# centreborelli/satnerf

Hardware: AMD Instinct MI355X
Metric: training rays/sec (64 samples/ray) (higher is better)
Workload: dtype bf16; 1 GPU; BASELINE configs[1] sat-nerf 256/tau4, 1024 rays x 64 samples/GPU, mlp_mode=bf16, saved state 8-bit, noise_std=0 sc_lambda=0 n_importance=0, stratified jitter drawn in-kernel (Philox-4x32-10); rays_per_gpu=1024, global_batch=1024, n_samples=64, parallelism=dp1

## Files before the change

include/satrender.h:

```cpp
#ifndef SATRENDER_H
#define SATRENDER_H

#include <stdint.h>

#ifdef __cplusplus
extern "C" {
#endif

#define SR_VERSION 100

#define SR_MODE_BF16 1
#define SR_MODE_BF16X3 3
#define SR_MODE_F16 2

#define SR_FMT16 16
#define SR_FMT8 8

int sr_version(void);
const char* sr_last_error(void);

int64_t sr_fwd_stream_elems(int feat, int tau);
int64_t sr_bwd_stream_elems(int feat, int tau);
int64_t sr_act_elems_per_tile(int feat, int fmt);
int64_t sr_dpre_elems_per_tile(int feat, int fmt);
// ... 49 lines not shown
  int tick;
  const float* noise;
  float noise_std;
  int sky_hidden;
  const float* sky_w1;
  const float* sky_b1;
  const float* sky_w2;
  const float* sky_b2;
  int64_t bank_chunks;
} sr_render_args;

typedef struct sr_render_outputs {
  float* z_vals;
  float* albedo;
  float* sigma;
  float* sun_v;
  float* beta;
  float* sky;
  float* weights;
  float* transparency;
  float* depth;
  float* rgb;
} sr_render_outputs;

int sr_satnerf_render_fwd(const sr_render_args* in, int feat, int tau, int mode, const uint16_t* stream_hi, const uint16_t* stream_lo,
                          const float* l0, const sr_render_outputs* out, void* stream);
int sr_render_points_per_block(int feat, int mode);

typedef struct sr_train_args {
  const float* target;
  const float* sched;
  float beta_min;
  float* loss_parts;
  float* rgb;
  float* d_sigma;
  float* d_albedo;
  float* d_sun_v;
  float* g_beta;
  float* d_sky;
  const int64_t* gather_idx;
  float* cursor;
  int64_t batches;
  float* out_rays;
  float* out_rgbs;
  int64_t* out_ts;
} sr_train_args;
int sr_satnerf_render_train(const sr_render_args* in, int feat, int tau, int mode, const uint16_t* stream_hi, const uint16_t* stream_lo,
                            const float* l0, const sr_render_outputs* out, const sr_train_args* train, uint16_t* acts, int act_fmt, void* stream);

int sr_satnerf_mlp_bwd(int feat, int tau, int64_t n_points, const uint16_t* bwd_stream, const uint16_t* acts,
                       const float* albedo, const float* sigma, const float* sun_v, const float* beta, const float* g_albedo,
                       const float* g_sigma, const float* g_sun_v, const float* g_beta, uint16_t* dpre, float* d_t, int fmt,
                       void* stream);
int sr_wgrad_plan(int32_t* blocks, int n_blocks, int64_t n_points, int n_wg, int fmt, int* n_slices);
int sr_satnerf_wgrad(int feat, int tau, int64_t n_points, const uint16_t* dpre, const uint16_t* acts, const int32_t* blocks,
                     int n_blocks, int n_slices, float* partial, void* stream);
int sr_satnerf_wgrad8(int feat, int tau, int64_t n_points, const uint16_t* dpre, int64_t dpre_elems, const uint16_t* acts,
                      const int32_t* blocks, const int32_t* loads, int n_blocks, int n_slices, int plan_span, float* partial, void* stream);
int sr_wgrad8_load_ints(void);

int sr_sky_bwd(const float* sun, int sun_stride, int64_t n, int hidden, const float* w1, const float* b1, const float* w2,
               const float* sky, const float* d_sky, float* g_w1, float* g_b1, float* g_w2, float* g_b2, void* stream);
int sr_embedding_bwd(const float* d_t, const int64_t* ts, int64_t n_rays, int n_samples, int tau, float* g_emb, void* stream);

int sr_sc_loss(const float* z_vals, const float* sigma, const float* noise, float noise_std, const float* sun_v, int64_t n_rays,
               int n_samples, float lambda_sc, float* loss_parts, float* d_sun_v, void* stream);
int sr_depth_loss(const float* depth, const float* depths, int depths_stride, int use_weights, int64_t n_rays, float lambda_ds,
                  float* loss_parts, float* g_depth, void* stream);
int sr_ray_setup(const float* rays, int ray_stride, const float* u, int64_t n_rays, int n_samples, int hidden, const float* w1,
                 const float* b1, const float* w2, const float* b2, float* z_vals, float* sky, void* stream);
int sr_ray_setup_rng(const float* rays, int ray_stride, uint64_t seed, float* step_counter, int tick, int64_t n_rays, int n_samples,
                     int hidden, const float* w1, const float* b1, const float* w2, const float* b2, float* z_vals, float* sky,
                     void* stream);
int sr_render_loss(const float* z_vals, const float* sigma, const float* noise, float noise_std, const float* albedo,
                   const float* sun_v, const float* beta, const float* sky, const float* target, int64_t n_rays, int n_samples,
                   float beta_min, const float* sched, float* loss_parts, float* rgb, float* d_sigma, float* d_albedo, float* d_sun_v,
                   float* g_beta, float* d_sky, void* stream);

int sr_grad_tail(const float* partial, const int32_t* gidx, const float* gscale, int64_t n_params, const int32_t* blocks, int n_blocks,
                 float* grad, int accumulate, const float* sun, int sun_stride, int64_t n_rays, int hidden,
                 const float* w1, const float* b1, const float* w2, const float* sky, const float* d_sky, float* g_w1, float* g_b1,
                 float* g_w2, float* g_b2, const float* d_t, const int64_t* ts, int n_samples, int tau, float* g_emb, void* stream);
typedef struct sr_pack_scatter {
  const int32_t* map;
  uint16_t* hi;
  uint16_t* lo;
  float* l0;
  int64_t n_f16;
  float scales[4];
} sr_pack_scatter;
int sr_grad_tail_adam(const float* partial, const int32_t* gidx, const float* gscale, int64_t n_params, const int32_t* blocks, int n_blocks,
                      float* grad,
                      int accumulate, const float* sun, int sun_stride, int64_t n_rays, int hidden, const float* w1, const float* b1,
                      const float* w2, const float* sky, const float* d_sky, float* g_w1, float* g_b1, float* g_w2, float* g_b2,
                      const float* d_t, const int64_t* ts, int n_samples, int tau, float* g_emb, float* params, float* exp_avg,
                      float* exp_avg_sq, const int32_t* late_idx, int n_late, float* state, float lr, float beta1, float beta2, float eps,
                      float grad_scale, const sr_pack_scatter* pack, void* stream);
int sr_adam_step_graph(float* params, float* grads, float* exp_avg, float* exp_avg_sq, int64_t n, float lr, float beta1,
                       float beta2, float eps, float grad_scale, float* state, int zero_grad, void* stream);
int sr_adam_step_pack(float* params, float* grads, float* exp_avg, float* exp_avg_sq, int64_t n, float lr, float beta1, float beta2,
                      float eps, float grad_scale, float* state, int zero_grad, int64_t n_packed, const sr_pack_scatter* pack,
                      void* stream);

enum { SR_ACT_NONE = 0, SR_ACT_SIN = 1, SR_ACT_RELU = 2 };
enum { SR_OUT_NONE = 0, SR_OUT_SOFTPLUS = 1, SR_OUT_SIGMOID = 2, SR_OUT_SIGMOID_RGB = 3 };
typedef struct sr_linear_src {
// ... 96 lines not shown
```

satnerf_amd/_lib.py:

```python
from __future__ import annotations

import ctypes as C
import os

_HERE = os.path.dirname(os.path.abspath(__file__))
LIB_PATH = os.environ.get("SATRENDER_LIB") or os.path.join(_HERE, "csrc", "libsatrender.so")

MODE_BF16 = 1
MODE_F16 = 2
MODE_BF16X3 = 3
FMT16, FMT8 = 16, 8

_vp, _i, _i64, _f, _d = C.c_void_p, C.c_int, C.c_int64, C.c_float, C.c_double


class MlpInputs(C.Structure):
    _fields_ = [("org", _vp), ("org_stride", _i), ("dir", _vp), ("dir_stride", _i), ("sun", _vp), ("sun_stride", _i),
                ("z", _vp), ("temb", _vp), ("ts", _vp), ("n_points", _i64), ("n_samples", _i)]


class RenderArgs(C.Structure):
    _fields_ = [("rays", _vp), ("ray_stride", _i), ("ts", _vp), ("temb", _vp), ("n_rays", _i64), ("n_samples", _i), ("z_in", _vp), ("u", _vp),
                ("seed", C.c_uint64), ("step_counter", _vp), ("tick", _i), ("noise", _vp), ("noise_std", _f), ("sky_hidden", _i),
                ("sky_w1", _vp), ("sky_b1", _vp), ("sky_w2", _vp), ("sky_b2", _vp), ("bank_chunks", _i64)]


class RenderOutputs(C.Structure):
    _fields_ = [(k, _vp) for k in ("z_vals", "albedo", "sigma", "sun_v", "beta", "sky", "weights", "transparency", "depth", "rgb")]


class TrainArgs(C.Structure):
    _fields_ = [("target", _vp), ("sched", _vp), ("beta_min", _f), ("loss_parts", _vp), ("rgb", _vp), ("d_sigma", _vp), ("d_albedo", _vp),
                ("d_sun_v", _vp), ("g_beta", _vp), ("d_sky", _vp), ("gather_idx", _vp), ("cursor", _vp), ("batches", _i64), ("out_rays", _vp),
                ("out_rgbs", _vp), ("out_ts", _vp)]


class PackScatter(C.Structure):
    _fields_ = [("map", _vp), ("hi", _vp), ("lo", _vp), ("l0", _vp), ("n_f16", _i64), ("scales", _f * 4)]


class LinearSrc(C.Structure):
    _fields_ = [("x", _vp), ("ld", _i), ("k", _i), ("act", _i), ("w0", _f), ("row_div", _i)]


ACT_NONE, ACT_SIN, ACT_RELU = 0, 1, 2
OUT_NONE, OUT_SOFTPLUS, OUT_SIGMOID, OUT_SIGMOID_RGB = 0, 1, 2, 3

SIGNATURES = {
    "sr_version": (_i, []),
    "sr_last_error": (C.c_char_p, []),
    "sr_fwd_stream_elems": (_i64, [_i, _i]),
    "sr_bwd_stream_elems": (_i64, [_i, _i]),
    "sr_act_elems_per_tile": (_i64, [_i, _i]),
    "sr_satnerf_render_fwd": (_i, [_vp, _i, _i, _i, _vp, _vp, _vp, _vp, _vp]),
    "sr_render_points_per_block": (_i, [_i, _i]),
    "sr_satnerf_render_train": (_i, [_vp, _i, _i, _i, _vp, _vp, _vp, _vp, _vp, _vp, _i, _vp]),
    "sr_pack_stream": (_i, [_vp, _vp, _vp, _i64, _vp, _vp, _i64, _vp]),
    "sr_dpre_elems_per_tile": (_i64, [_i, _i]),
    "sr_workspace_tiles": (_i64, [_i64]),
    "sr_dpre_workspace_elems": (_i64, [_i64, _i, _i]),
    "sr_unpack_grads": (_i, [_vp, _vp, _vp, _i64, _vp, _vp, _i, _vp]),
    "sr_composite_image": (_i, [_vp, _vp, _vp, _f, _vp, _vp, _vp, _vp, _i64, _i, _vp, _vp]),
    "sr_latlonalt_from_depth": (_i, [_vp, _i, _vp, _i64, _vp, _d, _vp, _vp, _vp, _vp]),
    "sr_linear_fwd": (_i, [C.POINTER(LinearSrc), _i, _vp, _vp, _i64, _i, _i, _vp, _i, _vp]),
    "sr_linear_bwd_input": (_i, [_vp, _i, _vp, _i, _i, _vp, _i, _i, C.POINTER(LinearSrc), _i64, _i, _vp, _i, _vp]),
    "sr_linear_bwd_weight": (_i, [_vp, _i, _vp, _i, _i, C.POINTER(LinearSrc), _i, _i64, _i, _vp, _vp, _vp]),
    "sr_positional_map": (_i, [_vp, _i, _i, _i64, _i, _vp, _vp]),
    "sr_points_along": (_i, [_vp, _i, _i, _vp, _i64, _i, _vp, _vp]),
    "sr_wgrad_plan": (_i, [_vp, _i, _i64, _i, _i, _vp]),
    "sr_satnerf_mlp_bwd": (_i, [_i, _i, _i64, _vp, _vp, _vp, _vp, _vp, _vp, _vp, _vp, _vp, _vp, _vp, _vp, _i, _vp]),
    "sr_satnerf_wgrad": (_i, [_i, _i, _i64, _vp, _vp, _vp, _i, _i, _vp, _vp]),
    "sr_satnerf_wgrad8": (_i, [_i, _i, _i64, _vp, _i64, _vp, _vp, _vp, _i, _i, _i, _vp, _vp]),
    "sr_wgrad8_load_ints": (_i, []),
    "sr_sky_bwd": (_i, [_vp, _i, _i64, _i, _vp, _vp, _vp, _vp, _vp, _vp, _vp, _vp, _vp, _vp]),
    "sr_embedding_bwd": (_i, [_vp, _vp, _i64, _i, _i, _vp, _vp]),
    "sr_ray_setup": (_i, [_vp, _i, _vp, _i64, _i, _i, _vp, _vp, _vp, _vp, _vp, _vp, _vp]),
    "sr_sc_loss": (_i, [_vp, _vp, _vp, _f, _vp, _i64, _i, _f, _vp, _vp, _vp]),
    "sr_depth_loss": (_i, [_vp, _vp, _i, _i, _i64, _f, _vp, _vp, _vp]),
    "sr_ray_setup_rng": (_i, [_vp, _i, C.c_uint64, _vp, _i, _i64, _i, _i, _vp, _vp, _vp, _vp, _vp, _vp, _vp]),
    "sr_render_loss": (_i, [_vp, _vp, _vp, _f, _vp, _vp, _vp, _vp, _vp, _i64, _i, _f, _vp, _vp, _vp, _vp, _vp, _vp, _vp, _vp, _vp]),
    "sr_satnerf_loss": (_i, [_vp, _vp, _vp, _vp, _i64, _i, _f, _f, _vp, _vp, _vp, _vp, _vp, _vp]),
    "sr_adam_step": (_i, [_vp, _vp, _vp, _vp, _i64, _f, _f, _f, _f, _f, _i64, _i, _vp]),
    "sr_gather_setup": (_i, [_vp, _vp, _vp, _vp, _i64, _vp, _vp, _vp, _vp, _i64, _i, _i, _vp, _vp, _vp, _vp, _vp, _vp, C.c_uint64, _vp, _i, _vp]),
    "sr_gather_batch": (_i, [_vp, _vp, _vp, _vp, _i64, _vp, _vp, _vp, _vp, _i64, _vp]),
    "sr_grad_tail": (_i, [_vp, _vp, _vp, _i64, _vp, _i, _vp, _i, _vp, _i, _i64, _i, _vp, _vp, _vp, _vp, _vp, _vp, _vp, _vp, _vp, _vp, _vp, _i, _i,
                          _vp, _vp]),
    "sr_grad_tail_adam": (_i, [_vp, _vp, _vp, _i64, _vp, _i, _vp, _i, _vp, _i, _i64, _i, _vp, _vp, _vp, _vp, _vp, _vp, _vp, _vp, _vp, _vp, _vp, _i, _i,
                               _vp, _vp, _vp, _vp, _vp, _i, _vp, _f, _f, _f, _f, _f, _vp, _vp]),
    "sr_adam_step_graph": (_i, [_vp, _vp, _vp, _vp, _i64, _f, _f, _f, _f, _f, _vp, _i, _vp]),
    "sr_adam_step_pack": (_i, [_vp, _vp, _vp, _vp, _i64, _f, _f, _f, _f, _f, _vp, _i, _i64, _vp, _vp]),
    "sr_pack_all": (_i, [_vp, _vp, _vp, _i64, _vp, _vp, _vp, _vp, _i64, _vp, _vp, _i64, _vp]),
    "sr_gather_scale_f32": (_i, [_vp, _vp, _vp, _i64, _vp, _vp]),
    "sr_ray_sample_fwd": (_i, [_vp, _i, _vp, _i64, _i, _vp, _vp]),
    "sr_sky_fwd": (_i, [_vp, _i, _i64, _i, _vp, _vp, _vp, _vp, _vp, _vp]),
    "sr_satnerf_mlp_fwd": (_i, [C.POINTER(MlpInputs), _i, _i, _i, _vp, _vp, _vp, _vp, _vp, _vp, _vp, _vp, _i, _vp]),
    "sr_composite_fwd": (_i, [_vp, _vp, _vp, _f, _vp, _vp, _vp, _i64, _i, _i, _vp, _vp, _vp, _vp, _vp]),
    "sr_composite_bwd": (_i, [_vp, _vp, _vp, _f, _vp, _vp, _vp, _vp, _vp, _vp, _i64, _i, _i, _vp, _vp, _vp, _vp, _vp, _vp,
                              _vp, _vp, _vp]),
    "sr_sample_pdf_merge": (_i, [_vp, _vp, _vp, _i64, _i, _i, _f, _vp, _vp]),
    "sr_sample_pdf": (_i, [_vp, _vp, _vp, _i64, _i, _i, _f, _vp, _vp]),
    "sr_rpc_rays": (_i, [_vp, _i, _i, _d, _d, _vp, _d, _d, _d, _vp, _vp, _vp]),
    "sr_rpc_rays_at": (_i, [_vp, _vp, _i64, _d, _d, _vp, _d, _d, _d, _vp, _vp]),
    "sr_reprojection_errors": (_i, [_vp, _vp, _vp, _i64, _vp, _i64, _vp, _vp]),
    "sr_keypoint_weights_scratch": (_i, [_i64, _i, C.POINTER(_i64)]),
    "sr_keypoint_weights": (_i, [_vp, _vp, _vp, _i64, _i64, _i, _vp, _i64, _vp, _vp, _vp, _vp]),
    "sr_tie_point_depths": (_i, [_vp, _vp, _vp, _i64, _i64, _vp, _d, _vp, _vp, _vp]),
    "sr_idw_grid_scratch": (_i, [_i64, _i, C.POINTER(_i64)]),
    "sr_idw_interpolate": (_i, [_vp, _vp, _i64, _vp, _i64, _i, _i, _i, _vp, _i64, _vp, _vp, _vp, _vp]),
    "sr_gaussian_filter_f64": (_i, [_vp, _i, _i, _vp, _i, _vp, _i, _vp, _vp, _vp]),
    "sr_utm_zone": (_i, [_d, _d, C.POINTER(_i), C.POINTER(_i)]),
    "sr_utm_from_latlon": (_i, [_vp, _vp, _i64, _i, _vp, _vp, _vp]),
    "sr_depth_to_utm": (_i, [_vp, _i, _vp, _i64, _vp, _d, _i, _vp, _vp, _vp, _vp, _vp]),
    "sr_dsm_bounds": (_i, [_vp, _vp, _vp, _i64, _vp, _vp]),
    "sr_dsm_rasterize": (_i, [_vp, _vp, _vp, _i64, _d, _d, _d, _i, _i, _i, _d, _vp, _vp, _vp, _vp]),
    "sr_dsm_register_scratch": (_i, [_i, _i, _i, _i, _i, C.POINTER(_i64), C.POINTER(_i)]),
    "sr_dsm_downsample2x": (_i, [_vp, _i, _i, _vp, _vp]),
    "sr_dsm_compute_shift": (_i, [_vp, _i, _i, _vp, _i, _i, _i, _i, _vp, _i64, _vp, _vp, _vp, _vp, _vp]),
    "sr_dsm_apply_shift": (_i, [_vp, _i, _i, _vp, _vp, _vp, _vp]),
    "sr_image_metrics_scratch": (_i, [_i64, _i64, _i, _i, C.POINTER(_i64)]),
    "sr_image_sse": (_i, [_vp, _vp, _i64, _vp, _i64, _vp, _i64, _vp, _vp]),
    "sr_ssim_sum": (_i, [_vp, _vp, _i64, _i, _i, _vp, _i64, _vp, _vp]),
# ... 30 lines not shown
```

satnerf_amd/csrc/mlp_bwd.hip:

```cpp
#ifndef SR_BWD_TILES
#define SR_BWD_TILES 1
#endif
#if SR_BWD_TILES == 2
#define SR_MODE1_NW 4
#endif
#include "mlp_bwd.inc"

namespace sr {
int launch_bwd512(const BwdParams& p, int fmt, hipStream_t st);
long bwd512_stream_pieces();
int dpre8_units_512();
int act8_units_512(int auxs);
}

using namespace sr;

extern "C" int sr_satnerf_mlp_bwd(int feat, int tau, int64_t n_points, const uint16_t* bwd_stream, const uint16_t* acts, const float* albedo,
                                  const float* sigma, const float* sun_v, const float* beta, const float* g_albedo, const float* g_sigma,
                                  const float* g_sun_v, const float* g_beta, uint16_t* dpre, float* d_t, int fmt, void* stream) {
  SR_REQUIRE(feat == kFeat || feat == 512, "sr_satnerf_mlp_bwd: feat=%d unsupported (this build handles %d and 512)", feat, kFeat);
  SR_REQUIRE(tau >= 1 && tau <= 24, "sr_satnerf_mlp_bwd: tau=%d unsupported (1..24)", tau);
  SR_REQUIRE(fmt == SR_FMT16 || fmt == SR_FMT8, "sr_satnerf_mlp_bwd: workspace format must be 16 or 8 (got %d)", fmt);
  SR_REQUIRE(feat == kFeat || fmt == SR_FMT8, "sr_satnerf_mlp_bwd: feat=512 trains on the 8-bit workspaces only");
  SR_REQUIRE(bwd_stream && acts && dpre && albedo && sigma && sun_v && beta, "sr_satnerf_mlp_bwd: null pointer argument");
  if (n_points <= 0) return 0;
  BwdParams p;
  p.g_albedo = g_albedo, p.g_sigma = g_sigma, p.g_sun = g_sun_v, p.g_beta = g_beta;
  p.albedo = albedo, p.sigma = sigma, p.sun_v = sun_v, p.beta = beta;
  p.acts = (const uint4*)acts, p.dpre = (uint4*)dpre, p.d_t = d_t;
  p.stream = (const char*)bwd_stream;
  p.n_points = n_points, p.tau = tau, p.auxs = aux_steps(tau);
  p.emax = fmt == SR_FMT8 ? (uint4*)(dpre + sr_workspace_tiles(n_points) * sr_dpre_elems_per_tile(feat, fmt)) : nullptr;
  if (feat == 512) return launch_bwd512(p, fmt, (hipStream_t)stream);
  return fmt == SR_FMT8 ? launch_bwd_fmt<SR_FMT8>(p, (hipStream_t)stream) : launch_bwd_fmt<SR_FMT16>(p, (hipStream_t)stream);
}

extern "C" int64_t sr_bwd_stream_elems(int feat, int tau) {
  if ((feat != kFeat && feat != 512) || tau < 1 || tau > 24) return -1;
  return (feat == 512 ? bwd512_stream_pieces() : BwdStream::total_pieces()) * 512;
}

extern "C" int64_t sr_workspace_tiles(int64_t n_points) { return n_points < 0 ? -1 : sr::ws_tiles(n_points); }

extern "C" int64_t sr_dpre_elems_per_tile(int feat, int fmt) {
  if (fmt != SR_FMT16 && fmt != SR_FMT8) return -1;
  if (feat == 512) return fmt == SR_FMT8 ? (int64_t)dpre8_units_512() * 64 * 8 : -1;
  if (feat != kFeat) return -1;
  return (int64_t)(fmt == SR_FMT8 ? kD8Units : kDpFrags) * 64 * 8;
}

extern "C" int64_t sr_dpre_workspace_elems(int64_t n_points, int feat, int fmt) {
  const int64_t per_tile = sr_dpre_elems_per_tile(feat, fmt);
  if (per_tile < 0 || n_points < 0) return -1;
  return sr::ws_tiles(n_points) * per_tile + (fmt == SR_FMT8 ? sr::ws_emax_bytes(n_points) / 2 : 0);
}

extern "C" int64_t sr_act_elems_per_tile(int feat, int fmt) {
  if (fmt != SR_FMT16 && fmt != SR_FMT8) return -1;
  if (feat == 512) return fmt == SR_FMT8 ? (int64_t)act8_units_512(2) * 64 * 8 : -1;
  if (feat != kFeat) return -1;
  return (int64_t)(fmt == SR_FMT8 ? act8_units(2) : act_ksteps(2)) * 64 * 8;
}
```

satnerf_amd/csrc/mlp_bwd.inc:

```
#pragma once
#include "mlp_device.h"
#include "mlp_params.h"
#include "codec8.h"

namespace sr {
inline namespace SR_FEAT_NS {

using BS = BwdStream;
constexpr int kBSlot = BS::SLOTP * 1024;
#ifndef SR_BWD_TILES
#define SR_BWD_TILES 1
#endif
constexpr int kBT = SR_BWD_TILES;

template <int G, int LIMIT>
__device__ __forceinline__ void bchunk_enter(char* ring, const char* stream, int wave, int lane) {
  constexpr int later = [] {
    int n = 0;
    for (int c = 1; c < kD; ++c) n += G + c < LIMIT ? min_loads<1>(BS::np(G + c)) : 0;
    return n;
  }();
  wait_then_barrier<later>();
  if constexpr (G + kD < LIMIT) {
    constexpr long off = BS::offset_pieces(G + kD) * 1024L;
// ... 89 lines not shown
template <int KIN>
__device__ __forceinline__ void btile(const char* slot, int p0, const uint4 (&in)[kBT][KIN], f32x16 (&acc)[kBT], int lane) {
#pragma unroll
  for (int j = 0; j < kBT; ++j) acc[j] = f32x16{0};
  uint4 a = {};
#pragma unroll
  for (int i = 0; i < KIN; ++i) {
#ifdef SR_ABL_HALF_LDS
    if (i % 2 == 0)
#endif
    a = *reinterpret_cast<const uint4*>(slot + (p0 + i) * 1024 + lane * 16);
#pragma unroll
    for (int j = 0; j < kBT; ++j) acc[j] = mfma(a, in[j][i], acc[j]);
  }
}
template <int NP, int OFF, int KIN>
__device__ __forceinline__ void btile_part(const char* slot, const uint4 (&in)[kBT][KIN], f32x16 (&acc)[kBT], int lane) {
#pragma unroll
  for (int i = 0; i < NP; ++i) {
    const uint4 a = *reinterpret_cast<const uint4*>(slot + i * 1024 + lane * 16);
#pragma unroll
    for (int j = 0; j < kBT; ++j) acc[j] = mfma(a, in[j][OFF + i], acc[j]);
  }
}

template <int NP, int NS, int NSS>
struct TrunkSched {
  static constexpr int ND = 2 * kKS / Mode<1>::NW;
  static constexpr int tile_len(int t) { return (t % 2 == 0 ? ND : 0) + NP + (t > 0 ? NS : 0); }
  static constexpr int tile_start(int t) {
    int p = 0;
    for (int k = 0; k < t; ++k) p += tile_len(k);
    return p;
  }
  static constexpr int period() { return tile_start(kMT) + NS + NSS; }
  static constexpr int after_d(int t) { return tile_start(t) + ND; }
  static constexpr int after_p(int t) { return tile_start(t) + (t % 2 == 0 ? ND : 0) + NP; }
  static constexpr int at_store(int t) { return t < kMT - 1 ? after_p(t + 1) : tile_start(kMT); }
  static constexpr int wait_b(int t) {
    if (t >= 2) return at_store(t) - after_p(t - 2);
    const int steady = at_store(t) - (after_p(t + kMT - 2) - period());
    const int first = t == 0 ? NP + at_store(0) : at_store(1);
    return steady < first ? steady : first;
  }
  static constexpr int wait_a(int t) { return t >= 2 ? tile_start(t) - after_d(t - 2) : tile_start(0) - (after_d(kMT - 2) - period()); }
};

template <int N>
__device__ __forceinline__ void wait_vmcnt() {
  static_assert(N >= 0 && N < 64, "vmcnt is a 6-bit field");
  asm volatile("s_waitcnt vmcnt(%0)" ::"n"(N) : "memory");
}

struct PreSched {
  static constexpr int kTiles = 3 * kMTH + kMTH + kMTH + kMT;
  static constexpr int frag(int k) {
    if (k < 3 * kMTH) {
      const int part = k / kMTH, t = k % kMTH;
      return (part == 0 ? kActRgbh : part == 1 ? kActS3 : kActE1) + 2 * t;
    }
    k -= 3 * kMTH;
    if (k < kMTH) return kActS2 + 2 * k;
    k -= kMTH;
    if (k < kMTH) return kActS1 + 2 * k;
    return kActA0 + 7 * kKS + 2 * (k - kMTH);
  }
  static constexpr int chunk_of(int k) {
    if (k < 3 * kMTH) return BS::G_H;
    k -= 3 * kMTH;
    if (k < kMTH) return BS::G_S3 + k / 2;
    k -= kMTH;
    if (k < kMTH) return BS::G_S2 + k / 2;
    return BS::G_G1 + (k - kMTH);
  }
  static constexpr int kAhead = 4;
  static constexpr int wait(int k, int nph, int limit) {
    int n = 0;
    const int req_chunk = k >= kAhead ? chunk_of(k - kAhead) : -1;
    for (int g = req_chunk + 1; g <= chunk_of(k); ++g) n += g + kD < limit ? min_loads<1>(BS::np(g + kD)) : 0;
    const int later = kTiles - 1 - k < kAhead - 1 ? kTiles - 1 - k : kAhead - 1;
    n += nph * later;
    return n < 63 ? n : 63;
  }
};

template <int FMT, int LIMIT, int KIN, int TPC, int NCHUNK, int G0, bool COS, int NOUT, int PK0, int DF0, class Req>
__device__ __forceinline__ void bstage(const uint4 (&in)[kBT][KIN], uint4 (&out)[kBT][NOUT], char* ring, const char* stream, int wave, int lane,
                                       const char* stage, Req&& request, uint4* const (&dpre_tile)[kBT], uint32_t* const (&emax)[kBT]) {
  constexpr int NPH = FMT == SR_FMT8 ? 1 : 2;
  uint32_t eb[kBT][4] = {};
  static_for<NCHUNK>([&](auto cc) {
    constexpr int c = decltype(cc)::value, g = G0 + c;
    static_assert(BS::np(g) == TPC * KIN, "backward stream geometry mismatch");
    bchunk_enter<g, LIMIT>(ring, stream, wave, lane);
    const char* slot = ring + (g % kNSLOT) * kBSlot;
    static_for<TPC>([&](auto tc) {
      constexpr int tt = decltype(tc)::value, t = c * TPC + tt, o = 2 * t;
      Phase<FMT> ph[kBT] = {};
      f32x16 acc[kBT];
      btile<KIN>(slot, tt * KIN, in, acc, lane);
      if constexpr (COS) {
        constexpr int k = PK0 + t;
        wait_vmcnt<PreSched::wait(k, kBT * NPH, LIMIT)>();
#pragma unroll
        for (int j = 0; j < kBT; ++j) ph[j].from_lds(stage + ((k & 3) * kBT + j) * NPH * 1024, lane);
      }
#pragma unroll
      for (int j = 0; j < kBT; ++j)
        eb[j][t >> 2] |= bpack<COS, FMT>(acc[j], ph[j], out[j][o], out[j][o + 1], dpre_tile[j], DF0 + 2 * t) << (8 * (t & 3));
      if constexpr (COS && PK0 + t + PreSched::kAhead < PreSched::kTiles) request((PK0 + t + PreSched::kAhead) & 3, PreSched::frag(PK0 + t + PreSched::kAhead));
    });
  });
#pragma unroll
  for (int j = 0; j < kBT; ++j) store_scales<FMT, TPC * NCHUNK>(dpre_tile[j], dp8_group(DF0), eb[j], emax[j]);
}

typedef uint32_t u32x32w __attribute__((ext_vector_type(32)));
typedef uint32_t u32x4w __attribute__((ext_vector_type(4)));
template <int FMT, bool TRUNK_ASM = false>
__global__ void __launch_bounds__(Mode<1>::NW * 64) satnerf_bwd_kernel(const BwdParams prm) {
  constexpr int NW = Mode<1>::NW;
  constexpr bool kStreamG1 = false;
  constexpr int LIMIT = !TRUNK_ASM ? BS::NCH : kStreamG1 ? BS::G_G1 : BS::G_L;
  extern __shared__ __attribute__((aligned(16))) char smem[];
  char* ring = smem;
#ifdef SR_BWD_TIMING
  const uint64_t t_kernel0 = __builtin_amdgcn_s_memtime(), r_kernel0 = __builtin_amdgcn_s_memrealtime();
#endif
  const int tid = threadIdx.x, lane = tid & 63;
  const int wave = __builtin_amdgcn_readfirstlane(tid >> 6);
  const int h = lane >> 5, pl = lane & 31;
  const char* stream = prm.stream;
  const int A = prm.auxs, AK = FMT == SR_FMT8 ? act8_units(prm.auxs) : act_ksteps(prm.auxs);
  constexpr int DK = FMT == SR_FMT8 ? kD8Units : kDpFrags;

#pragma unroll
  for (int g = 0; g < kD; ++g) {
    if (g == 0) issue_chunk<1, BS::np(0)>(stream, nullptr, 0, ring, wave, lane);
    if (g == 1) issue_chunk<1, BS::np(1)>(stream, nullptr, BS::offset_pieces(1) * 1024L, ring + kBSlot, wave, lane);
    if (g == 2) issue_chunk<1, BS::np(2)>(stream, nullptr, BS::offset_pieces(2) * 1024L, ring + 2 * kBSlot, wave, lane);
  }

#ifdef SR_BWD_REVERSE
  const long tile0 = ((long)(gridDim.x - 1 - blockIdx.x) * NW + wave) * kBT;
#else
  const long tile0 = ((long)blockIdx.x * NW + wave) * kBT;
#endif
  long pt[kBT];
  bool valid[kBT];
  uint4* dpre[kBT];
#pragma unroll
  for (int j = 0; j < kBT; ++j) {
    pt[j] = (tile0 + j) * 32 + pl;
    valid[j] = pt[j] < prm.n_points;
    dpre[j] = prm.dpre + (tile0 + j) * DK * 64 + lane;
  }

  uint4 dhead[kBT][1], dsig[kBT];
  uint32_t e_feats[kBT] = {}, e_raw[kBT] = {};
#pragma unroll
  for (int j = 0; j < kBT; ++j) {
    float v[8] = {0.f, 0.f, 0.f, 0.f, 0.f, 0.f, 0.f, 0.f}, sg = 0.f;
    const long q = pt[j];
    uint4 fs = {};
    if constexpr (FMT == SR_FMT8)
      fs = prm.acts[((tile0 + j) * (long)act8_units(prm.auxs) + prm.auxs + kA8Scale) * 64 + lane];
    if (valid[j]) {
      if (h == 0) {
        if (prm.g_albedo) {
#pragma unroll
          for (int c = 0; c < 3; ++c) {
            const float s = (prm.albedo[q * 3 + c] + 0.001f) * (1.0f / 1.002f);
            v[c] = prm.g_albedo[q * 3 + c] * 1.002f * s * (1.0f - s);
          }
        }
        if (prm.g_sun) {
          const float s = prm.sun_v[q];
          v[3] = prm.g_sun[q] * s * (1.0f - s);
        }
        if (prm.g_sigma) sg = prm.g_sigma[q] * (1.0f - expf(-prm.sigma[q]));
      } else if (prm.g_beta) {
        v[0] = prm.g_beta[q] * (1.0f - expf(-prm.beta[q]));
      }
    }
    dhead[j][0] = make_uint4(pack_bf16x2(v[0], v[1]), pack_bf16x2(v[2], v[3]), pack_bf16x2(v[4], v[5]), pack_bf16x2(v[6], v[7]));
    dsig[j] = make_uint4(pack_bf16x2(sg, 0.f), 0u, 0u, 0u);
    dpre[j][(FMT == SR_FMT8 ? kD8Head : kDpHead) * 64] = dhead[j][0];
    dpre[j][(FMT == SR_FMT8 ? kD8Sigma : kDpSigma) * 64] = dsig[j];
    if constexpr (FMT == SR_FMT8) {
      const uint32_t w4[4] = {fs.x, fs.y, kMT > 8 ? fs.z : 0u, kMT > 8 ? fs.w : 0u};
      e_feats[j] = max_byte<kMT>(w4);
      const uint32_t hw[5] = {dhead[j][0].x, dhead[j][0].y, dhead[j][0].z, dhead[j][0].w, dsig[j].x};
      uint32_t m = 0;
#pragma unroll
      for (int k = 0; k < 5; ++k) {
        const uint32_t lo = (hw[k] & 0x7fffu) >> 7, hi = (hw[k] >> 23) & 0xffu;
        m = m > lo ? m : lo, m = m > hi ? m : hi;
      }
      e_raw[j] = m;
    }
  }

  constexpr int NPH = FMT == SR_FMT8 ? 1 : 2;
  constexpr int NPT = kBT * NPH;
  char* stage = smem + kNSLOT * kBSlot + wave * (4 * NPT * 1024);
  const uint32_t stage_addr = __builtin_amdgcn_readfirstlane(lds_addr_of(stage));
  auto stage_phase = [&](int slot, int frag) {
#ifdef SR_ABL_NO_PHASE_LOADS
    return;
#endif
#pragma unroll
    for (int j = 0; j < kBT; ++j) {
      const char* src = reinterpret_cast<const char*>(prm.acts + ((tile0 + j) * AK + A + (FMT == SR_FMT8 ? frag >> 1 : frag)) * 64);
#pragma unroll
      for (int k = 0; k < NPH; ++k) glds16_s(src + k * 1024, (uint32_t)lane * 16u, stage_addr + ((slot * kBT + j) * NPH + k) * 1024);
    }
  };
  auto phases_of = [&](int slot, Phase<FMT> (&ph)[kBT]) {
#pragma unroll
    for (int j = 0; j < kBT; ++j) ph[j].from_lds(stage + (slot * kBT + j) * NPH * 1024, lane);
  };
  static_assert(PreSched::kAhead == 4, "the wave's phase staging ring has four slots");
  stage_phase(0, PreSched::frag(0)), stage_phase(1, PreSched::frag(1)), stage_phase(2, PreSched::frag(2)), stage_phase(3, PreSched::frag(3));

  uint32_t* emax_cells = reinterpret_cast<uint32_t*>(smem + kNSLOT * kBSlot + NW * (4 * NPT * 1024));
  uint32_t* emax[kBT];
#pragma unroll
  for (int j = 0; j < kBT; ++j) emax[j] = emax_cells + (wave * kBT + j) * 16;
  if constexpr (FMT == SR_FMT8) {
#pragma unroll
    for (int j = 0; j < kBT; ++j) note_emax(emax[j], kEmaxFeats, e_feats[j], lane), note_emax(emax[j], kEmaxRaw, e_raw[j], lane);
  }

#ifdef SR_BWD_TIMING
  uint64_t t_stage[5];
  t_stage[0] = __builtin_amdgcn_s_memtime();
#endif
  uint4 d_rgbh[kBT][kHS], d_s3[kBT][kHS], d_e1[kBT][kHS];
  {
    bchunk_enter<BS::G_H, LIMIT>(ring, stream, wave, lane);
    const char* slot = ring + (BS::G_H % kNSLOT) * kBSlot;
    uint32_t eb[kBT][3][4] = {};
    static_for<3 * kMTH>([&](auto tc) {
      constexpr int T = decltype(tc)::value, part = T / kMTH, t = T % kMTH;
      constexpr int dp0 = part == 0 ? kDpRgbh : (part == 1 ? kDpS3 : kDpE1);
      f32x16 acc[kBT];
      btile<1>(slot, T, dhead, acc, lane);
      wait_vmcnt<PreSched::wait(T, NPT, LIMIT)>();
      Phase<FMT> ph[kBT];
      phases_of(T & 3, ph);
#pragma unroll
      for (int j = 0; j < kBT; ++j) {
        uint4 o0, o1;
        eb[j][part][t >> 2] |= bpack<true, FMT>(acc[j], ph[j], o0, o1, dpre[j], dp0 + 2 * t) << (8 * (t & 3));
        if constexpr (part == 0) d_rgbh[j][2 * t] = o0, d_rgbh[j][2 * t + 1] = o1;
        else if constexpr (part == 1) d_s3[j][2 * t] = o0, d_s3[j][2 * t + 1] = o1;
        else d_e1[j][2 * t] = o0, d_e1[j][2 * t + 1] = o1;
      }
      stage_phase((T + PreSched::kAhead) & 3, PreSched::frag(T + PreSched::kAhead));
    });
#pragma unroll
    for (int j = 0; j < kBT; ++j) {
      store_scales<FMT, kMTH>(dpre[j], dp8_group(kDpRgbh), eb[j][0], emax[j]);
      store_scales<FMT, kMTH>(dpre[j], dp8_group(kDpS3), eb[j][1], emax[j]);
      store_scales<FMT, kMTH>(dpre[j], dp8_group(kDpE1), eb[j][2], emax[j]);
    }
  }
#ifdef SR_BWD_TIMING
  t_stage[1] = __builtin_amdgcn_s_memtime();
#endif
  uint4 d_g2[kBT][3 * kHS];
  {
    uint4 d_s2[kBT][kHS], d_s1[kBT][kHS];
    bstage<FMT, LIMIT, kHS, 2, kMTH / 2, BS::G_S3, true, kHS, 3 * kMTH, kDpS2>(d_s3, d_s2, ring, stream, wave, lane, stage, stage_phase, dpre, emax);
    bstage<FMT, LIMIT, kHS, 2, kMTH / 2, BS::G_S2, true, kHS, 4 * kMTH, kDpS1>(d_s2, d_s1, ring, stream, wave, lane, stage, stage_phase, dpre, emax);
#pragma unroll
    for (int j = 0; j < kBT; ++j) {
#pragma unroll
      for (int i = 0; i < kHS; ++i) d_g2[j][i] = d_rgbh[j][i], d_g2[j][kHS + i] = d_s1[j][i], d_g2[j][2 * kHS + i] = d_e1[j][i];
    }
  }
#ifdef SR_BWD_TIMING
  t_stage[2] = __builtin_amdgcn_s_memtime();
#endif
  uint4 d_g1[kBT][kKS + 1];
  {
    uint4 d_feats[kBT][kKS];
    {
      uint32_t eb[kBT][4] = {};
      static_for<kMT>([&](auto tc) {
        constexpr int t = decltype(tc)::value;
        f32x16 acc[kBT];
#pragma unroll
        for (int j = 0; j < kBT; ++j) acc[j] = f32x16{0};
        static_for<BS::kG2Split>([&](auto sc) {
          constexpr int sp = decltype(sc)::value, g = BS::G_G2 + t * BS::kG2Split + sp;
          static_assert(BS::np(g) == BS::kG2Part, "backward stream geometry mismatch");
          bchunk_enter<g, LIMIT>(ring, stream, wave, lane);
          btile_part<BS::kG2Part, sp * BS::kG2Part>(ring + (g % kNSLOT) * kBSlot, d_g2, acc, lane);
        });
        Phase<FMT> none = {};
#pragma unroll
        for (int j = 0; j < kBT; ++j)
          eb[j][t >> 2] |= bpack<false, FMT>(acc[j], none, d_feats[j][2 * t], d_feats[j][2 * t + 1], dpre[j], kDpFeats + 2 * t) << (8 * (t & 3));
      });
#pragma unroll
      for (int j = 0; j < kBT; ++j) store_scales<FMT, kMT>(dpre[j], dp8_group(kDpFeats), eb[j], emax[j]);
    }
    bchunk_enter<BS::G_DT, LIMIT>(ring, stream, wave, lane);
    f32x16 acc[kBT];
    btile<kHS>(ring + (BS::G_DT % kNSLOT) * kBSlot, 0, d_e1, acc, lane);
#pragma unroll
// ... 143 lines not shown
    wait_vmcnt<TS::wait_b(kMT - 1)>();
    epilogue(std::integral_constant<int, kMT - 1>{});
#pragma unroll
    for (int j = 0; j < kBT; ++j) {
      store_scales<FMT, kMT>(dpre[j], l - 1, eb[j], emax[j]);
#pragma unroll
      for (int i = 0; i < kKS; ++i) cur[j][i] = nxt[j][i];
    }
  }
#ifdef SR_BWD_TIMING
    if (lane == 0 && prm.d_t) {
      const uint64_t t_end = __builtin_amdgcn_s_memtime();
      prm.d_t[tile0 * 8 + 0] = (float)(t_stage[4] - t_kernel0), prm.d_t[tile0 * 8 + 1] = (float)(t_end - t_stage[4]);
      prm.d_t[tile0 * 8 + 2] = 1.f, prm.d_t[tile0 * 8 + 3] = 1.f;
      prm.d_t[tile0 * 8 + 4] = (float)(t_stage[0] - t_kernel0), prm.d_t[tile0 * 8 + 5] = (float)(t_stage[1] - t_stage[0]);
      prm.d_t[tile0 * 8 + 6] = (float)(t_stage[2] - t_stage[1]), prm.d_t[tile0 * 8 + 7] = (float)(t_stage[3] - t_stage[2]);
    }
#endif
  }
  if constexpr (FMT == SR_FMT8) {
    constexpr int kRows = NW * kBT, kEntries = (kRows + kEmaxTiles - 1) / kEmaxTiles;
    __syncthreads();
    if (tid < kEntries && prm.emax) {
      uint32_t w[4] = {0u, 0u, 0u, 0u};
#pragma unroll
      for (int g = 0; g < 16; ++g) {
        uint32_t m = 0;
#pragma unroll
        for (int r = 0; r < kEmaxTiles; ++r) {
          const int row = tid * kEmaxTiles + r;
          const uint32_t c = row < kRows ? emax_cells[row * 16 + g] : 0u;
          m = m > c ? m : c;
        }
        w[g >> 2] |= m << (8 * (g & 3));
      }
      prm.emax[(tile0 - (long)wave * kBT) / kEmaxTiles + tid] = make_uint4(w[0], w[1], w[2], w[3]);
    }
  }
}


template <int FMT, bool TRUNK_ASM>
int launch_bwd_kernel(const BwdParams& p, size_t lds, hipStream_t st) {
  constexpr int NW = Mode<1>::NW;
  if (!ensure_dynamic_lds((const void*)satnerf_bwd_kernel<FMT, TRUNK_ASM>, lds)) return 1;
  const long tiles = (p.n_points + 31) / 32;
  hipLaunchKernelGGL((satnerf_bwd_kernel<FMT, TRUNK_ASM>), dim3((unsigned)((tiles + NW * kBT - 1) / (NW * kBT))), dim3(NW * 64), lds, st, p);
  return check_launch("satnerf_bwd_kernel");
}

template <int FMT>
int launch_bwd_fmt(const BwdParams& p, hipStream_t st) {
  constexpr int NW = Mode<1>::NW;
  const size_t lds = (size_t)kNSLOT * kBSlot + NW * 4 * kBT * (FMT == SR_FMT8 ? 1 : 2) * 1024 + (FMT == SR_FMT8 ? NW * kBT * 64 : 0);
  if constexpr (FMT == SR_FMT8 && (kFeat == 256 || kFeat == 512) && kBT == 1) {
    const char* e = getenv("SATNERF_BWD_V1");
    const bool v1 = e && e[0] == '1';
    const unsigned long big = (unsigned long)ws_tiles(p.n_points) * (kD8Units > act8_units(2) ? kD8Units : act8_units(2)) * 1024ul;
    if (!v1 && big < (1ul << 32)) return launch_bwd_kernel<FMT, true>(p, lds, st);
  }
  return launch_bwd_kernel<FMT, false>(p, lds, st);
}

}
}
```

satnerf_amd/csrc/mlp_bwd512.hip:

```cpp
#define SR_FEAT 512
#include "mlp_bwd.inc"
namespace sr {
int launch_bwd512(const BwdParams& p, int fmt, hipStream_t st) {
  if (fmt != SR_FMT8) {
    set_error("sr_satnerf_mlp_bwd: feat=512 trains on the 8-bit workspaces only");
    return 1;
  }
  return launch_bwd_fmt<SR_FMT8>(p, st);
}
long bwd512_stream_pieces() { return BwdStream::total_pieces(); }
int dpre8_units_512() { return kD8Units; }
int act8_units_512(int auxs) { return act8_units(auxs); }
}
```

Measured before the change: 2.778 million rays/s.

## Deepen backward phase-staging prefetch ring to fill available LDS

Replaces the fixed 4-slot per-wave phase staging ring in the MLP backward kernel with a depth derived from the LDS budget left after the weight ring and exponent cells. Vmcnt wait counts are recomputed for the chosen depth, with a compile-time check that the 63 cap never drops a lead. The per-point head inputs and the 8-bit scale word are now loaded before the weight chunks are issued, so their latency overlaps the prefetch. Query entry points expose the depth, waits and LDS size. The trade-off is a larger LDS footprint per block, which can lower occupancy.

```diff
diff --git a/include/satrender.h b/include/satrender.h
--- a/include/satrender.h
+++ b/include/satrender.h
@@ -125,6 +125,10 @@
                        const float* albedo, const float* sigma, const float* sun_v, const float* beta, const float* g_albedo,
                        const float* g_sigma, const float* g_sun_v, const float* g_beta, uint16_t* dpre, float* d_t, int fmt,
                        void* stream);
+int sr_bwd_presched_wait(int feat, int fmt, int depth, int k);
+int sr_bwd_presched_depth(int feat, int fmt);
+int sr_bwd_presched_tiles(int feat, int fmt);
+int64_t sr_bwd_lds_bytes(int feat, int fmt);
 int sr_wgrad_plan(int32_t* blocks, int n_blocks, int64_t n_points, int n_wg, int fmt, int* n_slices);
 int sr_satnerf_wgrad(int feat, int tau, int64_t n_points, const uint16_t* dpre, const uint16_t* acts, const int32_t* blocks,
                      int n_blocks, int n_slices, float* partial, void* stream);
diff --git a/satnerf_amd/_lib.py b/satnerf_amd/_lib.py
--- a/satnerf_amd/_lib.py
+++ b/satnerf_amd/_lib.py
@@ -67,6 +67,10 @@
     "sr_linear_bwd_weight": (_i, [_vp, _i, _vp, _i, _i, C.POINTER(LinearSrc), _i, _i64, _i, _vp, _vp, _vp]),
     "sr_positional_map": (_i, [_vp, _i, _i, _i64, _i, _vp, _vp]),
     "sr_points_along": (_i, [_vp, _i, _i, _vp, _i64, _i, _vp, _vp]),
+    "sr_bwd_presched_wait": (_i, [_i, _i, _i, _i]),
+    "sr_bwd_presched_depth": (_i, [_i, _i]),
+    "sr_bwd_presched_tiles": (_i, [_i, _i]),
+    "sr_bwd_lds_bytes": (_i64, [_i, _i]),
     "sr_wgrad_plan": (_i, [_vp, _i, _i64, _i, _i, _vp]),
     "sr_satnerf_mlp_bwd": (_i, [_i, _i, _i64, _vp, _vp, _vp, _vp, _vp, _vp, _vp, _vp, _vp, _vp, _vp, _vp, _i, _vp]),
     "sr_satnerf_wgrad": (_i, [_i, _i, _i64, _vp, _vp, _vp, _i, _i, _vp, _vp]),
diff --git a/satnerf_amd/csrc/mlp_bwd.hip b/satnerf_amd/csrc/mlp_bwd.hip
--- a/satnerf_amd/csrc/mlp_bwd.hip
+++ b/satnerf_amd/csrc/mlp_bwd.hip
@@ -11,6 +11,7 @@
 long bwd512_stream_pieces();
 int dpre8_units_512();
 int act8_units_512(int auxs);
+int bwd512_presched_query(int what, int depth, int k);
 }
 
 using namespace sr;
@@ -40,6 +41,16 @@
   return (feat == 512 ? bwd512_stream_pieces() : BwdStream::total_pieces()) * 512;
 }
 
+static int presched(int feat, int fmt, int what, int depth, int k) {
+  if (feat == 512) return fmt == SR_FMT8 ? bwd512_presched_query(what, depth, k) : -1;
+  if (feat != kFeat) return -1;
+  return fmt == SR_FMT8 ? presched_query<SR_FMT8>(what, depth, k) : fmt == SR_FMT16 ? presched_query<SR_FMT16>(what, depth, k) : -1;
+}
+extern "C" int sr_bwd_presched_wait(int feat, int fmt, int depth, int k) { return presched(feat, fmt, 0, depth, k); }
+extern "C" int sr_bwd_presched_depth(int feat, int fmt) { return presched(feat, fmt, 1, 0, 0); }
+extern "C" int sr_bwd_presched_tiles(int feat, int fmt) { return presched(feat, fmt, 3, 0, 0); }
+extern "C" int64_t sr_bwd_lds_bytes(int feat, int fmt) { return presched(feat, fmt, 2, 0, 0); }
+
 extern "C" int64_t sr_workspace_tiles(int64_t n_points) { return n_points < 0 ? -1 : sr::ws_tiles(n_points); }
 
 extern "C" int64_t sr_dpre_elems_per_tile(int feat, int fmt) {
diff --git a/satnerf_amd/csrc/mlp_bwd.inc b/satnerf_amd/csrc/mlp_bwd.inc
--- a/satnerf_amd/csrc/mlp_bwd.inc
+++ b/satnerf_amd/csrc/mlp_bwd.inc
@@ -165,8 +165,11 @@
   asm volatile("s_waitcnt vmcnt(%0)" ::"n"(N) : "memory");
 }
 
+template <int FMT>
 struct PreSched {
   static constexpr int kTiles = 3 * kMTH + kMTH + kMTH + kMT;
+  static constexpr int NW = Mode<1>::NW;
+  static constexpr int NPT = kBT * (FMT == SR_FMT8 ? 1 : 2);
   static constexpr int frag(int k) {
     if (k < 3 * kMTH) {
       const int part = k / kMTH, t = k % kMTH;
@@ -186,20 +189,50 @@
     if (k < kMTH) return BS::G_S2 + k / 2;
     return BS::G_G1 + (k - kMTH);
   }
-  static constexpr int kAhead = 4;
-  static constexpr int wait(int k, int nph, int limit) {
+  static constexpr int kLdsLimit = 160 * 1024;
+  static constexpr int kEmaxBytes = FMT == SR_FMT8 ? NW * kBT * 64 : 0;
+#ifdef SR_BWD_PHASE_AHEAD
+  static constexpr int kAhead = SR_BWD_PHASE_AHEAD;
+#else
+  static constexpr int kAhead = (kLdsLimit - kNSLOT * kBSlot - kEmaxBytes) / (NW * NPT * 1024);
+#endif
+  static constexpr int kStageBytes = kAhead * NPT * 1024;
+  static constexpr int kLdsBytes = kNSLOT * kBSlot + NW * kStageBytes + kEmaxBytes;
+  static_assert(kAhead >= 4 && kAhead <= kTiles, "the compiler-scheduled trunk cycles through slots 0..3 of the same staging ring");
+  static_assert(kLdsBytes <= kLdsLimit, "weight ring + phase staging + exponent-maxima cells exceed the LDS");
+  static constexpr int loads_after(int ahead, int k, int limit) {
     int n = 0;
-    const int req_chunk = k >= kAhead ? chunk_of(k - kAhead) : -1;
+    const int req_chunk = k >= ahead ? chunk_of(k - ahead) : -1;
     for (int g = req_chunk + 1; g <= chunk_of(k); ++g) n += g + kD < limit ? min_loads<1>(BS::np(g + kD)) : 0;
-    const int later = kTiles - 1 - k < kAhead - 1 ? kTiles - 1 - k : kAhead - 1;
-    n += nph * later;
+    const int later = kTiles - 1 - k < ahead - 1 ? kTiles - 1 - k : ahead - 1;
+    return n + NPT * later;
+  }
+  static constexpr int wait_at(int ahead, int k, int limit) {
+    const int n = loads_after(ahead, k, limit);
     return n < 63 ? n : 63;
+  }
+  static constexpr int wait(int k, int limit) { return wait_at(kAhead, k, limit); }
+  static constexpr int max_loads(int np) { return (np + NW - 1) / NW; }
+  static constexpr bool lead_kept(int ahead, int k, int limit) {
+    if (loads_after(ahead, k, limit) < 63) return true;
+    const int c = chunk_of(k);
+    int n = 0, used = 0;
+    for (int g = c + 1; g < c + kD; ++g) n += g < limit ? min_loads<1>(BS::np(g)) : 0;
+    n = n < 63 ? n : 63;
+    for (int q = 0; q < k; ++q) used += chunk_of(q) == c;
+    return n + (c + kD < limit ? max_loads(BS::np(c + kD)) : 0) + NPT * used <= 63;
+  }
+  static constexpr bool all_leads_kept(int limit) {
+    for (int k = 0; k < kTiles; ++k)
+      if (!lead_kept(kAhead, k, limit)) return false;
+    return true;
   }
 };
 
 template <int FMT, int LIMIT, int KIN, int TPC, int NCHUNK, int G0, bool COS, int NOUT, int PK0, int DF0, class Req>
 __device__ __forceinline__ void bstage(const uint4 (&in)[kBT][KIN], uint4 (&out)[kBT][NOUT], char* ring, const char* stream, int wave, int lane,
                                        const char* stage, Req&& request, uint4* const (&dpre_tile)[kBT], uint32_t* const (&emax)[kBT]) {
+  using PS = PreSched<FMT>;
   constexpr int NPH = FMT == SR_FMT8 ? 1 : 2;
   uint32_t eb[kBT][4] = {};
   static_for<NCHUNK>([&](auto cc) {
@@ -214,14 +247,14 @@
       btile<KIN>(slot, tt * KIN, in, acc, lane);
       if constexpr (COS) {
         constexpr int k = PK0 + t;
-        wait_vmcnt<PreSched::wait(k, kBT * NPH, LIMIT)>();
-#pragma unroll
-        for (int j = 0; j < kBT; ++j) ph[j].from_lds(stage + ((k & 3) * kBT + j) * NPH * 1024, lane);
+        wait_vmcnt<PS::wait(k, LIMIT)>();
+#pragma unroll
+        for (int j = 0; j < kBT; ++j) ph[j].from_lds(stage + ((k % PS::kAhead) * kBT + j) * NPH * 1024, lane);
       }
 #pragma unroll
       for (int j = 0; j < kBT; ++j)
         eb[j][t >> 2] |= bpack<COS, FMT>(acc[j], ph[j], out[j][o], out[j][o + 1], dpre_tile[j], DF0 + 2 * t) << (8 * (t & 3));
-      if constexpr (COS && PK0 + t + PreSched::kAhead < PreSched::kTiles) request((PK0 + t + PreSched::kAhead) & 3, PreSched::frag(PK0 + t + PreSched::kAhead));
+      if constexpr (COS && PK0 + t + PS::kAhead < PS::kTiles) request((PK0 + t + PS::kAhead) % PS::kAhead, PS::frag(PK0 + t + PS::kAhead));
     });
   });
 #pragma unroll
@@ -247,13 +280,6 @@
   const int A = prm.auxs, AK = FMT == SR_FMT8 ? act8_units(prm.auxs) : act_ksteps(prm.auxs);
   constexpr int DK = FMT == SR_FMT8 ? kD8Units : kDpFrags;
 
-#pragma unroll
-  for (int g = 0; g < kD; ++g) {
-    if (g == 0) issue_chunk<1, BS::np(0)>(stream, nullptr, 0, ring, wave, lane);
-    if (g == 1) issue_chunk<1, BS::np(1)>(stream, nullptr, BS::offset_pieces(1) * 1024L, ring + kBSlot, wave, lane);
-    if (g == 2) issue_chunk<1, BS::np(2)>(stream, nullptr, BS::offset_pieces(2) * 1024L, ring + 2 * kBSlot, wave, lane);
-  }
-
 #ifdef SR_BWD_REVERSE
   const long tile0 = ((long)(gridDim.x - 1 - blockIdx.x) * NW + wave) * kBT;
 #else
@@ -269,31 +295,80 @@
     dpre[j] = prm.dpre + (tile0 + j) * DK * 64 + lane;
   }
 
+  float hv[kBT][12];
+  uint4 fs[kBT];
+#pragma unroll
+  for (int j = 0; j < kBT; ++j) {
+    const long q = valid[j] ? pt[j] : 0;
+    fs[j] = uint4{};
+    if constexpr (FMT == SR_FMT8) fs[j] = prm.acts[((tile0 + j) * (long)act8_units(prm.auxs) + prm.auxs + kA8Scale) * 64 + lane];
+    const float *ga = prm.g_albedo ? prm.g_albedo : prm.albedo, *gs = prm.g_sun ? prm.g_sun : prm.sun_v;
+    const float *gg = prm.g_sigma ? prm.g_sigma : prm.sigma, *gb = prm.g_beta ? prm.g_beta : prm.beta;
+#pragma unroll
+    for (int c = 0; c < 3; ++c) hv[j][c] = prm.albedo[q * 3 + c], hv[j][3 + c] = ga[q * 3 + c];
+    hv[j][6] = prm.sun_v[q], hv[j][7] = gs[q];
+    hv[j][8] = prm.sigma[q], hv[j][9] = gg[q];
+    hv[j][10] = prm.beta[q], hv[j][11] = gb[q];
+  }
+
+  constexpr long off1 = BS::offset_pieces(1) * 1024L, off2 = BS::offset_pieces(2) * 1024L;
+#pragma unroll
+  for (int g = 0; g < kD; ++g) {
+    if (g == 0) issue_chunk<1, BS::np(0)>(stream, nullptr, 0, ring, wave, lane);
+    if (g == 1) issue_chunk<1, BS::np(1)>(stream, nullptr, off1, ring + kBSlot, wave, lane);
+    if (g == 2) issue_chunk<1, BS::np(2)>(stream, nullptr, off2, ring + 2 * kBSlot, wave, lane);
+  }
+
+  using PS = PreSched<FMT>;
+  constexpr int NPH = FMT == SR_FMT8 ? 1 : 2;
+  constexpr int NPT = PS::NPT;
+  static_assert(PS::all_leads_kept(LIMIT), "a pre-trunk vmcnt saturates at 63 where loads can still be in flight: the extra lead would be lost");
+  char* stage = smem + kNSLOT * kBSlot + wave * PS::kStageBytes;
+  const uint32_t stage_addr = __builtin_amdgcn_readfirstlane(lds_addr_of(stage));
+  auto stage_phase = [&](int slot, int frag) {
+#ifdef SR_ABL_NO_PHASE_LOADS
+    return;
+#endif
+#pragma unroll
+    for (int j = 0; j < kBT; ++j) {
+      const char* src = reinterpret_cast<const char*>(prm.acts + ((tile0 + j) * AK + A + (FMT == SR_FMT8 ? frag >> 1 : frag)) * 64);
+#pragma unroll
+      for (int k = 0; k < NPH; ++k) glds16_s(src + k * 1024, (uint32_t)lane * 16u, stage_addr + ((slot * kBT + j) * NPH + k) * 1024);
+    }
+  };
+  auto phases_of = [&](int slot, Phase<FMT> (&ph)[kBT]) {
+#pragma unroll
+    for (int j = 0; j < kBT; ++j) ph[j].from_lds(stage + (slot * kBT + j) * NPH * 1024, lane);
+  };
+  static_for<PS::kAhead>([&](auto kc) { stage_phase(decltype(kc)::value, PS::frag(decltype(kc)::value)); });
+#pragma unroll
+  for (int j = 0; j < kBT; ++j) {
+#pragma unroll
+    for (int c = 0; c < 12; ++c) asm volatile("" : "+v"(hv[j][c]));
+    asm volatile("" : "+v"(fs[j].x), "+v"(fs[j].y), "+v"(fs[j].z), "+v"(fs[j].w));
+  }
+
   uint4 dhead[kBT][1], dsig[kBT];
   uint32_t e_feats[kBT] = {}, e_raw[kBT] = {};
 #pragma unroll
   for (int j = 0; j < kBT; ++j) {
     float v[8] = {0.f, 0.f, 0.f, 0.f, 0.f, 0.f, 0.f, 0.f}, sg = 0.f;
-    const long q = pt[j];
-    uint4 fs = {};
-    if constexpr (FMT == SR_FMT8)
-      fs = prm.acts[((tile0 + j) * (long)act8_units(prm.auxs) + prm.auxs + kA8Scale) * 64 + lane];
     if (valid[j]) {
       if (h == 0) {
         if (prm.g_albedo) {
 #pragma unroll
           for (int c = 0; c < 3; ++c) {
-            const float s = (prm.albedo[q * 3 + c] + 0.001f) * (1.0f / 1.002f);
-            v[c] = prm.g_albedo[q * 3 + c] * 1.002f * s * (1.0f - s);
+            const float s = (hv[j][c] + 0.001f) * (1.0f / 1.002f);
+            v[c] = hv[j][3 + c] * 1.002f * s * (1.0f - s);
           }
         }
         if (prm.g_sun) {
-          const float s = prm.sun_v[q];
-          v[3] = prm.g_sun[q] * s * (1.0f - s);
+          const float s = hv[j][6];
+          v[3] = hv[j][7] * s * (1.0f - s);
         }
-        if (prm.g_sigma) sg = prm.g_sigma[q] * (1.0f - expf(-prm.sigma[q]));
+        if (prm.g_sigma) sg = hv[j][9] * (1.0f - expf(-hv[j][8]));
       } else if (prm.g_beta) {
-        v[0] = prm.g_beta[q] * (1.0f - expf(-prm.beta[q]));
+        v[0] = hv[j][11] * (1.0f - expf(-hv[j][10]));
       }
     }
     dhead[j][0] = make_uint4(pack_bf16x2(v[0], v[1]), pack_bf16x2(v[2], v[3]), pack_bf16x2(v[4], v[5]), pack_bf16x2(v[6], v[7]));
@@ -301,7 +376,7 @@
     dpre[j][(FMT == SR_FMT8 ? kD8Head : kDpHead) * 64] = dhead[j][0];
     dpre[j][(FMT == SR_FMT8 ? kD8Sigma : kDpSigma) * 64] = dsig[j];
     if constexpr (FMT == SR_FMT8) {
-      const uint32_t w4[4] = {fs.x, fs.y, kMT > 8 ? fs.z : 0u, kMT > 8 ? fs.w : 0u};
+      const uint32_t w4[4] = {fs[j].x, fs[j].y, kMT > 8 ? fs[j].z : 0u, kMT > 8 ? fs[j].w : 0u};
       e_feats[j] = max_byte<kMT>(w4);
       const uint32_t hw[5] = {dhead[j][0].x, dhead[j][0].y, dhead[j][0].z, dhead[j][0].w, dsig[j].x};
       uint32_t m = 0;
@@ -314,29 +389,7 @@
     }
   }
 
-  constexpr int NPH = FMT == SR_FMT8 ? 1 : 2;
-  constexpr int NPT = kBT * NPH;
-  char* stage = smem + kNSLOT * kBSlot + wave * (4 * NPT * 1024);
-  const uint32_t stage_addr = __builtin_amdgcn_readfirstlane(lds_addr_of(stage));
-  auto stage_phase = [&](int slot, int frag) {
-#ifdef SR_ABL_NO_PHASE_LOADS
-    return;
-#endif
-#pragma unroll
-    for (int j = 0; j < kBT; ++j) {
-      const char* src = reinterpret_cast<const char*>(prm.acts + ((tile0 + j) * AK + A + (FMT == SR_FMT8 ? frag >> 1 : frag)) * 64);
-#pragma unroll
-      for (int k = 0; k < NPH; ++k) glds16_s(src + k * 1024, (uint32_t)lane * 16u, stage_addr + ((slot * kBT + j) * NPH + k) * 1024);
-    }
-  };
-  auto phases_of = [&](int slot, Phase<FMT> (&ph)[kBT]) {
-#pragma unroll
-    for (int j = 0; j < kBT; ++j) ph[j].from_lds(stage + (slot * kBT + j) * NPH * 1024, lane);
-  };
-  static_assert(PreSched::kAhead == 4, "the wave's phase staging ring has four slots");
-  stage_phase(0, PreSched::frag(0)), stage_phase(1, PreSched::frag(1)), stage_phase(2, PreSched::frag(2)), stage_phase(3, PreSched::frag(3));
-
-  uint32_t* emax_cells = reinterpret_cast<uint32_t*>(smem + kNSLOT * kBSlot + NW * (4 * NPT * 1024));
+  uint32_t* emax_cells = reinterpret_cast<uint32_t*>(smem + kNSLOT * kBSlot + NW * PS::kStageBytes);
   uint32_t* emax[kBT];
 #pragma unroll
   for (int j = 0; j < kBT; ++j) emax[j] = emax_cells + (wave * kBT + j) * 16;
@@ -359,9 +412,9 @@
       constexpr int dp0 = part == 0 ? kDpRgbh : (part == 1 ? kDpS3 : kDpE1);
       f32x16 acc[kBT];
       btile<1>(slot, T, dhead, acc, lane);
-      wait_vmcnt<PreSched::wait(T, NPT, LIMIT)>();
+      wait_vmcnt<PS::wait(T, LIMIT)>();
       Phase<FMT> ph[kBT];
-      phases_of(T & 3, ph);
+      phases_of(T % PS::kAhead, ph);
 #pragma unroll
       for (int j = 0; j < kBT; ++j) {
         uint4 o0, o1;
@@ -370,7 +423,7 @@
         else if constexpr (part == 1) d_s3[j][2 * t] = o0, d_s3[j][2 * t + 1] = o1;
         else d_e1[j][2 * t] = o0, d_e1[j][2 * t + 1] = o1;
       }
-      stage_phase((T + PreSched::kAhead) & 3, PreSched::frag(T + PreSched::kAhead));
+      if constexpr (T + PS::kAhead < PS::kTiles) stage_phase((T + PS::kAhead) % PS::kAhead, PS::frag(T + PS::kAhead));
     });
 #pragma unroll
     for (int j = 0; j < kBT; ++j) {
@@ -620,7 +673,7 @@
 template <int FMT>
 int launch_bwd_fmt(const BwdParams& p, hipStream_t st) {
   constexpr int NW = Mode<1>::NW;
-  const size_t lds = (size_t)kNSLOT * kBSlot + NW * 4 * kBT * (FMT == SR_FMT8 ? 1 : 2) * 1024 + (FMT == SR_FMT8 ? NW * kBT * 64 : 0);
+  const size_t lds = PreSched<FMT>::kLdsBytes;
   if constexpr (FMT == SR_FMT8 && (kFeat == 256 || kFeat == 512) && kBT == 1) {
     const char* e = getenv("SATNERF_BWD_V1");
     const bool v1 = e && e[0] == '1';
@@ -630,5 +683,16 @@
   return launch_bwd_kernel<FMT, false>(p, lds, st);
 }
 
-}
-}
+template <int FMT>
+int presched_query(int what, int depth, int k) {
+  using PS = PreSched<FMT>;
+  constexpr int limit = FMT == SR_FMT8 && kBT == 1 ? BS::G_L : BS::NCH;
+  if (what == 1) return PS::kAhead;
+  if (what == 2) return PS::kLdsBytes;
+  if (what == 3) return PS::kTiles;
+  if (what != 0 || k < 0 || k >= PS::kTiles || depth > PS::kTiles) return -1;
+  return PS::wait_at(depth > 0 ? depth : PS::kAhead, k, limit);
+}
+
+}
+}
diff --git a/satnerf_amd/csrc/mlp_bwd512.hip b/satnerf_amd/csrc/mlp_bwd512.hip
--- a/satnerf_amd/csrc/mlp_bwd512.hip
+++ b/satnerf_amd/csrc/mlp_bwd512.hip
@@ -11,4 +11,5 @@
 long bwd512_stream_pieces() { return BwdStream::total_pieces(); }
 int dpre8_units_512() { return kD8Units; }
 int act8_units_512(int auxs) { return act8_units(auxs); }
+int bwd512_presched_query(int what, int depth, int k) { return presched_query<SR_FMT8>(what, depth, k); }
 }
```

Result: no change. 2.760 million rays/s (-0.6%).
